# cvxgrp/qcqp

Measured on AMD Instinct MI355X. Metric: restarts x coord-sweeps / sec (improve COORD_DESCENT phase-2 sweeps, 2n^2 flops each; whole step timed), higher is better.
Workload: dtype f64

## Files before the change

### qcqp_amd/csrc/capi.hip

```cpp
#include <dlfcn.h>
#include <unistd.h>
#include <hip/hip_runtime.h>
#include <rccl/rccl.h>

#include <algorithm>
#include <cmath>
#include <cstdarg>
#include <cstdio>
#include <cstring>
#include <string>
#include <chrono>
#include <vector>

#include "../../include/qcqp_mi.h"
#include "kernels_impl.h"
#include "admm.h"
#include "admm_fused.h"
#include "cd_queue.h"
#include "cd_life.h"
#include "cd_small.h"
#include "admm_small.h"
#include "sdr_small.h"
#include "gemm_pk.h"
#include "cd_general.h"
// ... 112 lines not shown
    size_t h_pin_cap = 0;
    int64_t out_cap = 0;
    int eval_zs = 1;
    double *d_wS = nullptr, *d_wY = nullptr, *d_ww = nullptr, *d_wz = nullptr;
    int64_t wY_cap = 0;
    double *d_planes = nullptr;
    int64_t planes_cap = 0;
    double *d_gP = nullptr;
    const double *dn_Gpack = nullptr, *dn_q = nullptr, *dn_qT = nullptr, *dn_r = nullptr;
    const int *dn_relop = nullptr;
    double *dn_G = nullptr, *dn_Dg = nullptr, *dn_Ft = nullptr;
    int dense_chain_mode = 0;
    long long *dn_prof = nullptr;
    int64_t dn_G_cap = 0, dn_state_cap = 0;
    void *dn_state = nullptr;
    hipStream_t stream2 = nullptr;
    hipEvent_t dn_ev[3] = {nullptr, nullptr, nullptr};
    hipEvent_t dn_evn[2] = {nullptr, nullptr};
    int *dn_hn = nullptr;
    bool dn_force = false;
    double stream_limit = 16e9;
    double *dn_gp_pre = nullptr, *dn_tmp = nullptr;
    ncclComm_t comm = nullptr;
    int rank = 0, world = 1;
    double *d_comm = nullptr, *d_comm_big = nullptr;
    size_t comm_big_cap = 0;
    long long *d_prof = nullptr;
    int cd_stage = 0;
    int64_t Xi_cap = 0;
    bool sdr_factor_resident = false;
    double ad_Minv_rho = 0.0;
    bool ad_Minv_device = false;
    const char *last_cd2_kernel = "";
    bool profile = false;
    int dbg = 0;
    char *af_work = nullptr;
    size_t af_work_cap = 0;
    bool ad_fused = true;
    int ad_fused_nt = 512;
    const char *last_admm_kernel = "";
    int last_admm_C = 0;
    long long af_prof[16] = {0};
    int cd_queue = 2;
    int *d_qnext = nullptr;
    bool q_prepared = false;
    CdLife *d_life = nullptr;
    int Kreal = 0;
    double fbound = 0.0;
    double *l2_scratch = nullptr; size_t l2_scratch_cap = 0;
    double *l2_D = nullptr, *l2_S = nullptr;
    int *l2_abort = nullptr;
    int *l2_cuslot = nullptr;
    double *l2_preslack = nullptr; int64_t l2_preslack_cap = 0;
    double *lr_L = nullptr, *lr_G = nullptr, *lr_U = nullptr; int lr_RB = 0;
    int life_version = 0;
    long long *d_life_prof = nullptr;
    int64_t *d_bestK_idx = nullptr; double *d_bestK_key = nullptr, *d_bestK_x = nullptr; int64_t bestK_cap = 0;
    bool cd_ref_order = false;
    bool force_generic = false;
    std::vector<int> last_st1, last_st2;
    char *sb_work = nullptr;
    size_t sb_work_cap = 0;
    std::vector<double> unit_d;
    char *ss_work = nullptr;
    size_t ss_work_cap = 0;
};

namespace {

void admm_free(qcqpmi_ctx *c, bool keep_zsolver);

int fail(qcqpmi_ctx *c, int code, const char *fmt, ...) {
    char buf[1024];
    va_list ap;
    va_start(ap, fmt);
    vsnprintf(buf, sizeof(buf), fmt, ap);
    va_end(ap);
    if (c) c->err = buf; else g_create_error = buf;
    return code;
}

#define HIPCHK(c, expr)                                                                       \
    do {                                                                                      \
        hipError_t e_ = (expr);                                                               \
        if (e_ != hipSuccess)                                                                 \
            return fail(c, QCQPMI_EHIP, "%s failed: %s (%s:%d)", #expr, hipGetErrorString(e_), \
                        __FILE__, __LINE__);                                                  \
    } while (0)

template <typename T>
int dev_alloc(qcqpmi_ctx *c, T **p, size_t count, bool zero = true) {
    void *v = nullptr;
    HIPCHK(c, hipMalloc(&v, std::max<size_t>(count, 1) * sizeof(T)));
    if (zero) HIPCHK(c, hipMemsetAsync(v, 0, std::max<size_t>(count, 1) * sizeof(T), c->stream));
    *p = (T *)v;
    return 0;
}

template <typename T>
int prob_upload(qcqpmi_ctx *c, const T **dst, const std::vector<T> &src) {
    T *p = nullptr;
    int rc = dev_alloc(c, &p, src.size(), false);
    if (rc) return rc;
    c->prob_allocs.push_back(p);
    if (!src.empty())
        HIPCHK(c, hipMemcpyAsync(p, src.data(), src.size() * sizeof(T), hipMemcpyHostToDevice, c->stream));
// ... 425 lines not shown
}

#include "capi_small.inc"


extern "C" {

int qcqpmi_abi_version(void) { return QCQPMI_ABI_VERSION; }

int qcqpmi_device_count(void) {
    int n = 0;
    if (hipGetDeviceCount(&n) != hipSuccess) return 0;
    return n;
}

const char *qcqpmi_last_error(const qcqpmi_ctx *ctx) {
    return ctx ? ctx->err.c_str() : g_create_error.c_str();
}

int qcqpmi_ctx_create(qcqpmi_ctx **out, int64_t n, int64_t m, int device) {
    if (!out || n <= 0 || m < 0) return fail(nullptr, QCQPMI_EINVAL, "ctx_create: bad arguments");
    int ndev = qcqpmi_device_count();
    if (ndev <= 0)
        return fail(nullptr, QCQPMI_EHIP, "no HIP device visible: the qcqp_amd engine requires an MI355X (there is no CPU fallback)");
    if (device < 0 || device >= ndev) return fail(nullptr, QCQPMI_EINVAL, "device %d out of range (%d visible)", device, ndev);
    qcqpmi_ctx *c = new qcqpmi_ctx();
    c->device = device; c->n = n; c->m = m; c->n16 = (n + 15) / 16 * 16;
    c->quads.resize((size_t)m + 1);
    if (const char *sl = getenv("QCQPMI_STREAM_LIMIT")) { const double v = atof(sl); if (v > 0.0) c->stream_limit = v; }
    hipError_t e = hipSetDevice(device);
    if (e == hipSuccess) e = hipStreamCreateWithFlags(&c->stream, hipStreamNonBlocking);
    for (int i = 0; i < 5 && e == hipSuccess; i++) {
        e = hipEventCreate(&c->timers[i].beg);
        if (e == hipSuccess) e = hipEventCreate(&c->timers[i].end);
    }
    if (e != hipSuccess) {
        int rc = fail(nullptr, QCQPMI_EHIP, "ctx_create: %s", hipGetErrorString(e));
        delete c;
        return rc;
    }
    *out = c;
    return 0;
}

void qcqpmi_ctx_destroy(qcqpmi_ctx *c) {
    if (!c) return;
    (void)hipSetDevice(c->device);
    if (c->stream) (void)spin_sync(c->stream);
    if (c->comm && rccl() && rccl()->CommDestroy) rccl()->CommDestroy(c->comm);
    free_population(c);
    admm_free(c, false);
    for (void *p : c->prob_allocs) (void)hipFree(p);
    void *ptrs[] = {c->d_Fpack, c->d_Frow, c->d_mu, c->d_best_idx, c->d_best_key, c->d_comm, c->d_comm_big,
                    c->dn_G, c->dn_Dg, c->dn_Ft, c->dn_prof, c->dn_state, c->d_planes, c->d_out, c->d_wS, c->d_wY, c->d_ww, c->d_wz, c->af_work, c->d_qnext, c->d_life, c->d_life_prof, c->d_bestK_idx, c->d_bestK_key, c->d_bestK_x, c->l2_scratch, c->l2_D, c->l2_S, c->l2_abort, c->l2_cuslot, c->l2_preslack, c->lr_L, c->lr_G, c->lr_U, c->sb_work, c->ss_work};
    if (c->h_out) (void)hipHostFree(c->h_out);
    if (c->h_pin) (void)hipHostFree(c->h_pin);
    for (void *p : ptrs) if (p) (void)hipFree(p);
    for (auto &t : c->timers) { if (t.beg) (void)hipEventDestroy(t.beg); if (t.end) (void)hipEventDestroy(t.end); }
    for (auto &e : c->dn_ev) if (e) (void)hipEventDestroy(e);
    for (auto &e : c->dn_evn) if (e) (void)hipEventDestroy(e);
    if (c->dn_hn) (void)hipHostFree(c->dn_hn);
    if (c->stream2) (void)hipStreamDestroy(c->stream2);
    if (c->stream) (void)hipStreamDestroy(c->stream);
    delete c;
}

int qcqpmi_set_quad(qcqpmi_ctx *c, int64_t k, int format, const double *vals, const int64_t *idx,
                    const int64_t *ptr, int64_t nnz, const double *q, double r, int relop) {
    if (!c) return QCQPMI_EINVAL;
    if (c->finalized) return fail(c, QCQPMI_ESTATE, "set_quad after finalize");
    if (k < 0 || k > c->m || !q) return fail(c, QCQPMI_EINVAL, "set_quad: bad k or q");
    if ((k == 0) != (relop == 0) || relop < 0 || relop > 2)
        return fail(c, QCQPMI_EINVAL, "set_quad: relop %d invalid for function %lld", relop, (long long)k);
    HostQuad &h = c->quads[(size_t)k];
    h = HostQuad();
    const int64_t n = c->n;
    if (format == QCQPMI_FMT_DENSE) {
        if (!vals) return fail(c, QCQPMI_EINVAL, "set_quad: dense vals missing");
        for (int64_t i = 0; i < n; i++)
            for (int64_t j = 0; j < n; j++) {
                double v = vals[i * n + j];
                if (v != 0.0) { h.ci.push_back((int)i); h.cj.push_back((int)j); h.cv.push_back(v); }
            }
    } else if (format == QCQPMI_FMT_CSR) {
        if (!ptr || (nnz > 0 && (!idx || !vals))) return fail(c, QCQPMI_EINVAL, "set_quad: CSR arrays missing");
        for (int64_t i = 0; i < n; i++)
            for (int64_t e = ptr[i]; e < ptr[i + 1]; e++) {
                if (idx[e] < 0 || idx[e] >= n || e >= nnz) return fail(c, QCQPMI_EINVAL, "set_quad: CSR index out of range");
                if (vals[e] != 0.0) { h.ci.push_back((int)i); h.cj.push_back((int)idx[e]); h.cv.push_back(vals[e]); }
            }
    } else {
        return fail(c, QCQPMI_EINVAL, "set_quad: unknown format %d", format);
    }
    if (format == QCQPMI_FMT_DENSE) {
        for (int64_t i = 0; i < n; i++)
            for (int64_t j = i + 1; j < n; j++)
                if (vals[i * n + j] != vals[j * n + i])
                    return fail(c, QCQPMI_EINVAL, "set_quad: P of function %lld is not symmetric (entry %lld,%lld); pass (P + P^T)/2",
                                (long long)k, (long long)i, (long long)j);
    } else {
        std::vector<std::pair<int64_t, double>> ent(h.cv.size());
        for (size_t e = 0; e < h.cv.size(); e++) ent[e] = {(int64_t)h.ci[e] * n + h.cj[e], h.cv[e]};
        std::sort(ent.begin(), ent.end(), [](const std::pair<int64_t, double> &a, const std::pair<int64_t, double> &b) { return a.first < b.first; });
        size_t w = 0;
        for (size_t e = 0; e < ent.size(); e++) {
            if (w > 0 && ent[w - 1].first == ent[e].first) ent[w - 1].second += ent[e].second;
            else ent[w++] = ent[e];
// ... 653 lines not shown
            a.prof = c->d_prof;
        }
        bool used_rs = false;
        a.f0out = c->d_f0; a.mvout = c->d_mv;
        rc = (c->maxc <= 1) ? launch_cd<1>(c, a, false, used_lds, &used_rs) : launch_cd<4>(c, a, false, used_lds, &used_rs);
        if (rc) return rc;
        if (!used_rs && (rc = launch_eval(c, false))) return rc;
        if (stage == 2) { c->cd_stage = 2; return 0; }
    }
    c->cd_stage = 0;
    std::vector<int> st, st1;
    if ((rc = fetch_cd_outputs(c, sweeps1, sweeps2, visits2, accepted2, ran_phase2, f0, maxviol, st, st1))) return rc;
    if ((rc = cd_apply_status(c, st, st1, f0, maxviol, 0))) return rc;
    return 0;
}

int qcqpmi_cd_run(qcqpmi_ctx *c, int phase1, int64_t num_iters, double viol_tol, double tol,
                  uint64_t seed, uint64_t first_index, int64_t *sweeps1, int64_t *sweeps2,
                  int64_t *visits2, int64_t *accepted2, uint8_t *ran_phase2, double *f0,
                  double *maxviol) {
    return qcqpmi_cd_run_stage(c, 0, phase1, num_iters, viol_tol, tol, seed, first_index, sweeps1, sweeps2, visits2, accepted2,
                               ran_phase2, f0, maxviol);
}

int qcqpmi_cd_dense_block_step(qcqpmi_ctx *c, int phase, int64_t sweep, int64_t block, int coord_lo, int coord_hi, double viol_tol,
                               double tol, uint64_t seed, uint64_t first_index, const double *slack) {
    int rc = check_ready(c, true);
    if (rc) return rc;
    if (!dense_on(c)) return fail(c, QCQPMI_EUNSUPPORTED, "cd_dense_block_step: the problem does not take the dense-constraint path");
    c->last_cd2_kernel = dense_chain_name(c);
    return cd_dense_block_step(c, phase, sweep, block, coord_lo, coord_hi, viol_tol, tol, seed, first_index, slack);
}

static int cd_life2_reserve(qcqpmi_ctx *c, int nmw, int cus) {
    int rc;
    const size_t need = (size_t)cd_life2_max_wgs(nmw, cus, 1) * (size_t)c->n16 * 16;
    if (need > c->l2_scratch_cap) {
        if (c->l2_scratch) { HIPCHK(c, spin_sync(c->stream)); (void)hipFree(c->l2_scratch); c->l2_scratch = nullptr; c->l2_scratch_cap = 0; }
        if ((rc = dev_alloc(c, &c->l2_scratch, need))) return rc;
        c->l2_scratch_cap = need;
    }
    if (!c->l2_abort && (rc = dev_alloc(c, &c->l2_abort, 4))) return rc;
    if (!c->l2_cuslot && (rc = dev_alloc(c, &c->l2_cuslot, 4096))) return rc;
    if (!c->l2_D) {
        const size_t NB = (size_t)(c->n16 / 16);
        if ((rc = dev_alloc(c, &c->l2_D, NB * 256))) return rc;
        if ((rc = dev_alloc(c, &c->l2_S, NB * 48))) return rc;
        hipError_t e = (hipError_t)cd_life2_pack(c->dp, c->l2_D, c->l2_S, c->stream);
        if (e != hipSuccess) return fail(c, QCQPMI_EHIP, "cd_life2_pack: %s", hipGetErrorString(e));
    }
    return 0;
}

int qcqpmi_cd_stream_run(qcqpmi_ctx *c, int64_t K, int64_t R, int generate, int phase1, int64_t num_iters, double viol_tol, double tol,
                         uint64_t seed, uint64_t seed_stride, uint64_t first_index, uint64_t first_stride, double select_tol,
                         int64_t *sweeps1, int64_t *sweeps2, int64_t *visits2, int64_t *accepted2, uint8_t *ran_phase2, double *f0,
                         double *maxviol, int64_t *best_index, double *best_f0, double *best_maxviol, double *best_x) {
    int rc = check_ready(c, generate ? false : true);
    if (rc) return rc;
    if (K < 1 || R < 1 || num_iters < 0 || !(tol > 0.0) || K * R >= (1LL << 30)) return fail(c, QCQPMI_EINVAL, "cd_stream_run: bad K / R / num_iters / tol");
    if (!generate && c->R != K * R) return fail(c, QCQPMI_EINVAL, "cd_stream_run: the resident population has %lld points, K R = %lld", (long long)c->R, (long long)(K * R));
    HIPCHK(c, hipSetDevice(c->device));
    const bool stt = getenv("QCQPMI_STREAM_TIMING") != nullptr;
    double stm[6] = {0, 0, 0, 0, 0, 0};
    auto stnow = []() { return std::chrono::duration<double, std::milli>(std::chrono::steady_clock::now().time_since_epoch()).count(); };
    stm[0] = stnow();
    int nmw = 0, cs2 = 0, kind = 0;
    const int factor_rb = (c->lr_RB > 0 && c->life_version != 3 && cd_life2_factor_ok(c->dp, 16 * (int64_t)c->lr_RB)) ? c->lr_RB : 0;
    bool use2 = c->life_version != 1 && !c->force_generic && !(c->dbg & 64) && c->sep &&
                cd_life2_config(c->dp, c->Kreal, c->objclass, c->symcls, factor_rb, &nmw, &cs2, &kind);
    int cs = 0;
    const int queue_switch = c->cd_queue;
    c->cd_queue = 2;
    const bool eligible = cd_queue_eligible(c, false) && (int)(c->n16 / 16) - 4 <= RQ_NSIMD * RQ_MAXU && c->n16 >= 48;
    c->cd_queue = queue_switch;
    const bool lr = use2 && factor_rb > 0 && nmw == 3 && (kind == L2_KIND_BAND || kind == L2_KIND_GEN);
    if (lr) cs2 = 0;
    if (!use2) {
        if (!eligible || c->life_version != 1)
            return fail(c, QCQPMI_EUNSUPPORTED, "cd_stream_run: the lifecycle kernel needs separable constraints -- at most four classes of coordinates, at most two constraints "
                        "per coordinate --, a diagonal of P0 that is positive everywhere or zero everywhere (a diagonal of mixed sign: ONE class with one constraint "
                        "per coordinate only; with several classes or two constraints per coordinate it runs the serial path), and 33 <= n <= 2304: use qcqpmi_cd_run "
                        "per population");
        const int NBq = (int)(c->n16 / 16);
        cs = (c->dbg & 128) ? ((c->dbg >> 8) & 7) : 4;
        cs = cs > RQ_CSMAX ? RQ_CSMAX : cs;
        if (cs >= NBq) cs = 0;
        cs &= ~1;
        if (NBq - cs > RQ_NSIMD * RQ_MAXU || NBq < 3) return fail(c, QCQPMI_EUNSUPPORTED, "cd_stream_run: n = %lld outside the range of cd_phase2_qs_kernel (n <= 1024, at least 3 blocks of 16)", (long long)c->n);
    }
    if (generate && (rc = pop_reserve(c, K * R))) return rc;
    if (!c->d_qnext && (rc = dev_alloc(c, &c->d_qnext, 16))) return rc;
    if (!c->d_life) HIPCHK(c, hipMalloc((void **)&c->d_life, sizeof(CdLife)));
    HIPCHK(c, hipMemsetAsync(c->d_qnext, 0, 16 * sizeof(int), c->stream));
    CdLife L;
    L.on = 1; L.generate = generate ? 1 : 0; L.phase1 = phase1 ? 1 : 0; L.Rtotal = K * R; L.Rpop = R;
    L.seed = seed; L.seed_stride = seed_stride; L.first_index = first_index; L.first_stride = first_stride; L.viol_tol = viol_tol;
    L.sweeps1 = c->d_sweeps1; L.status1 = c->d_status1; L.ran2 = c->d_flag;
    L.prof = nullptr;
    const char *pre_ev = getenv("QCQPMI_L2_PREBUILT");
    const bool pre = lr && !(pre_ev && atoi(pre_ev) == 0);
    L.prebuilt = pre ? 1 : 0; L.preslack = nullptr;
    if (pre) {
        if (K * R > c->l2_preslack_cap) {
            if (c->l2_preslack) { HIPCHK(c, spin_sync(c->stream)); (void)hipFree(c->l2_preslack); c->l2_preslack = nullptr; c->l2_preslack_cap = 0; }
            if ((rc = dev_alloc(c, &c->l2_preslack, (size_t)(K * R)))) return rc;
            c->l2_preslack_cap = K * R;
        }
        L.preslack = c->l2_preslack;
    }
    if (c->profile) {
        if (!c->d_life_prof) HIPCHK(c, hipMalloc((void **)&c->d_life_prof, 24 * sizeof(long long)));
        HIPCHK(c, hipMemsetAsync(c->d_life_prof, 0, 24 * sizeof(long long), c->stream));
        L.prof = c->d_life_prof;
    }
    HIPCHK(c, hipMemcpyAsync(c->d_life, &L, sizeof(L), hipMemcpyHostToDevice, c->stream));
    HIPCHK(c, spin_sync(c->stream));
    int cus = 0;
    HIPCHK(c, hipDeviceGetAttribute(&cus, hipDeviceAttributeMultiprocessorCount, c->device));
    stm[1] = stnow();
    if (use2) {
        if ((rc = cd_life2_reserve(c, nmw, cus))) return rc;
        if (!lr && (c->dbg & 128)) { const int k2 = (c->dbg >> 8) & 7; if (nmw == 3 && (k2 == 0 || k2 == 2 || k2 == 4) && k2 < (int)(c->n16 / 16)) cs2 = k2; }
        const int tiles = cd_life2_tiles(c->dp, nmw, cs2, K * R, cus, 0, lr ? 1 : 0);
        int64_t wgs = (K * R + 16 * tiles - 1) / (16 * tiles);
        const int maxw = cd_life2_max_wgs(nmw, cus, tiles);
        if (wgs > maxw) wgs = maxw;
        if (c->dbg & 1024) { const int lim = (c->dbg >> 12) & 1023; if (lim > 0 && wgs > lim) wgs = lim; }
        CdLife2Args qa;
        qa.P = c->dp; qa.num_iters = num_iters; qa.tol = tol; qa.life = c->d_life;
        cd_queue_fill_batch(c, qa.b, seed, first_index);
        qa.b.R = K * R;
        qa.scratch = c->l2_scratch; qa.Dpack = c->l2_D; qa.Spack = c->l2_S; qa.abort = c->l2_abort; qa.fbound = c->fbound;
        { const char *ev = getenv("QCQPMI_L2_ROT"); const int rot = ev ? atoi(ev) : (lr ? 2 : 0); qa.cuslot = rot ? c->l2_cuslot : nullptr; qa.rotmode = rot; }
        if (qa.cuslot) HIPCHK(c, hipMemsetAsync(c->l2_cuslot, 0, 4096 * sizeof(int), c->stream));
        qa.dbg = (c->dbg & 2048) ? 1 : 0;
        qa.Gpack = lr ? c->lr_G : nullptr; qa.Upack = lr ? c->lr_U : nullptr; qa.RB = lr ? c->lr_RB : 0;
        qa.nclass = c->Kreal;
        const double l0 = stnow();
        (void)hipEventRecord(c->timers[2].beg, c->stream);
        const double l1 = stnow();
        hipError_t qe = pre ? (hipError_t)cd_life2_prep_launch(c->dp, c->d_life, c->X, K * R, num_iters, tol, c->stream) : hipSuccess;
        if (qe == hipSuccess) qe = (hipError_t)cd_life2_launch(qa, nmw, cs2, kind, tiles, (int)wgs, c->stream);
        const double l2 = stnow();
        (void)hipEventRecord(c->timers[2].end, c->stream);
        c->timers[2].valid = true;
        if (qe != hipSuccess) return fail(c, QCQPMI_EHIP, "cd_stream_run: %s", hipGetErrorString(qe));
        c->last_cd2_kernel = cd_life2_name(nmw, kind, tiles, lr ? 1 : 0);
        int ab = 0;
        HIPCHK(c, spin_sync(c->stream));
        const double l3 = stnow();
        HIPCHK(c, hipMemcpyAsync(&ab, c->l2_abort, sizeof(int), hipMemcpyDeviceToHost, c->stream));
        const double l4 = stnow();
        HIPCHK(c, spin_sync(c->stream));
        if (stt) fprintf(stderr, "cd_stream_run launch (ms): reserve %.3f, event %.3f, launch call %.3f, event + spin wait %.3f, copy call %.3f, sync %.3f\n", l0 - stm[1], l1 - l0, l2 - l1, l3 - l2, l4 - l3, stnow() - l4);
        if (ab) {
            HIPCHK(c, hipMemsetAsync(c->l2_abort, 0, sizeof(int), c->stream));
            c->R = 0;
            return fail(c, QCQPMI_EHIP, "cd_stream_run: a wait inside cd_life_kernel ran into its watchdog (internal error; no results)");
        }
    } else {
        CdQueueArgs qa;
        qa.P = c->dp; qa.num_iters = num_iters; qa.tol = tol;
        qa.life = c->d_life; qa.life_on = 1;
        cd_queue_fill_batch(c, qa.b, seed, first_index);
        qa.b.R = K * R;
        (void)hipEventRecord(c->timers[2].beg, c->stream);
        hipError_t qe = (hipError_t)cd_queue_launch(qa, cs, cus, c->stream);
        (void)hipEventRecord(c->timers[2].end, c->stream);
        c->timers[2].valid = true;
        if (qe != hipSuccess) return fail(c, QCQPMI_EHIP, "cd_stream_run: %s", hipGetErrorString(qe));
        HIPCHK(c, spin_sync(c->stream));
        c->last_cd2_kernel = "cd_phase2_qs_kernel<lifecycle>";
    }
    c->cd_stage = 0;
    c->evaluated = true;
    if (stt) { (void)spin_sync(c->stream); stm[2] = stnow(); }
    std::vector<int> st, st1;
    if ((rc = fetch_cd_outputs(c, sweeps1, sweeps2, visits2, accepted2, ran_phase2, f0, maxviol, st, st1))) return rc;
    stm[3] = stnow();
    if ((rc = cd_apply_status(c, st, st1, f0, maxviol, 0))) return rc;
    stm[4] = stnow();
    if (best_index || best_f0 || best_maxviol || best_x) {
        if ((rc = cd_bestK_reserve(c, K))) return rc;
        hipLaunchKernelGGL(select_best_kernel, dim3((unsigned)K), dim3(1024), 0, c->stream, (const double *)c->d_f0, (const double *)c->d_mv,
                           R, select_tol, c->d_bestK_idx, c->d_bestK_key);
        if (best_x) {
            HIPCHK(c, hipMemsetAsync(c->d_bestK_x, 0, (size_t)K * c->n * sizeof(double), c->stream));
            hipLaunchKernelGGL(gather_best_x_kernel, dim3((unsigned)K), dim3(256), 0, c->stream, (const double *)c->X, c->n, c->n16, R,
                               (const int64_t *)c->d_bestK_idx, c->d_bestK_x);
        }
        HIPCHK(c, hipGetLastError());
        std::vector<int64_t> idx((size_t)K * 2);
        std::vector<double> key((size_t)K * 2);
        HIPCHK(c, hipMemcpyAsync(idx.data(), c->d_bestK_idx, idx.size() * sizeof(int64_t), hipMemcpyDeviceToHost, c->stream));
        HIPCHK(c, hipMemcpyAsync(key.data(), c->d_bestK_key, key.size() * sizeof(double), hipMemcpyDeviceToHost, c->stream));
        if (best_x) HIPCHK(c, hipMemcpyAsync(best_x, c->d_bestK_x, (size_t)K * c->n * sizeof(double), hipMemcpyDeviceToHost, c->stream));
        HIPCHK(c, spin_sync(c->stream));
        for (int64_t p = 0; p < K; p++) {
            if (best_index) best_index[p] = idx[(size_t)2 * p];
            if (best_f0) best_f0[p] = key[(size_t)2 * p];
            if (best_maxviol) best_maxviol[p] = key[(size_t)2 * p + 1];
        }
    }
    if (stt) {
        stm[5] = stnow();
        fprintf(stderr, "cd_stream_run timing (ms): set-up %.3f, launch + kernel %.3f, fetch %.3f, status %.3f, best %.3f\n", stm[1] - stm[0], stm[2] - stm[1],
                stm[3] - stm[2], stm[4] - stm[3], stm[5] - stm[4]);
    }
    return 0;
}

int qcqpmi_cd_stream_reserve(qcqpmi_ctx *c, int64_t K, int64_t R) {
    int rc = check_ready(c, false);
    if (rc) return rc;
    if (K < 1 || R < 1 || K * R >= (1LL << 30)) return fail(c, QCQPMI_EINVAL, "cd_stream_reserve: bad K / R");
    HIPCHK(c, hipSetDevice(c->device));
    if (K * R > c->Rcap) { if ((rc = pop_reserve(c, K * R))) return rc; }
    if ((rc = cd_outputs_reserve(c, K * R))) return rc;
    if ((rc = cd_bestK_reserve(c, K))) return rc;
    if (!c->d_qnext && (rc = dev_alloc(c, &c->d_qnext, 16))) return rc;
    if (!c->d_life) HIPCHK(c, hipMalloc((void **)&c->d_life, sizeof(CdLife)));
    {
        int nmw = 0, cs2 = 0, kind = 0, cus = 0;
        HIPCHK(c, hipDeviceGetAttribute(&cus, hipDeviceAttributeMultiprocessorCount, c->device));
        if (c->life_version != 1 && c->sep && cd_life2_config(c->dp, c->Kreal, c->objclass, c->symcls, c->lr_RB, &nmw, &cs2, &kind) && (rc = cd_life2_reserve(c, nmw, cus))) return rc;
    }
    return 0;
}

int qcqpmi_debug_life_profile(qcqpmi_ctx *c, int64_t *out16) {
    if (!c || !out16) return QCQPMI_EINVAL;
    for (int k = 0; k < 24; k++) out16[k] = 0;
    if (!c->d_life_prof) return 0;
    HIPCHK(c, hipSetDevice(c->device));
    HIPCHK(c, spin_sync(c->stream));
    HIPCHK(c, hipMemcpy(out16, c->d_life_prof, 24 * sizeof(long long), hipMemcpyDeviceToHost));
    return 0;
}

int qcqpmi_cd_status(qcqpmi_ctx *c, int *status1, int *status2) {
    if (!c) return QCQPMI_EINVAL;
    if ((int64_t)c->last_st1.size() != c->R || (int64_t)c->last_st2.size() != c->R)
        return fail(c, QCQPMI_ESTATE, "cd_status: no coordinate-descent run on the resident population");
    if (status1) memcpy(status1, c->last_st1.data(), (size_t)c->R * sizeof(int));
    if (status2) memcpy(status2, c->last_st2.data(), (size_t)c->R * sizeof(int));
    return 0;
}


int qcqpmi_select_best(qcqpmi_ctx *c, double tol, int64_t *best_index, double *best_f0,
                       double *best_maxviol, double *best_x) {
    int rc = check_ready(c, true);
    if (rc) return rc;
    HIPCHK(c, hipSetDevice(c->device));
    if (!c->evaluated && (rc = launch_eval(c, false))) return rc;
    hipLaunchKernelGGL(select_best_kernel, dim3(1), dim3(1024), 0, c->stream, c->d_f0, c->d_mv, c->R, tol,
                       c->d_best_idx, c->d_best_key);
    HIPCHK(c, hipGetLastError());
    int64_t idx[2];
    double key[2];
    HIPCHK(c, hipMemcpyAsync(idx, c->d_best_idx, sizeof(idx), hipMemcpyDeviceToHost, c->stream));
    HIPCHK(c, hipMemcpyAsync(key, c->d_best_key, sizeof(key), hipMemcpyDeviceToHost, c->stream));
    HIPCHK(c, spin_sync(c->stream));
    if (best_index) *best_index = idx[0];
    if (best_f0) *best_f0 = key[0];
    if (best_maxviol) *best_maxviol = key[1];
    if (best_x && idx[0] >= 0) {
        int64_t r = idx[0];
        const double *src = c->X + (r >> 4) * c->n16 * 16 + (r & 15);
        HIPCHK(c, hipMemcpy2DAsync(best_x, sizeof(double), src, 16 * sizeof(double), sizeof(double), (size_t)c->n,
                                   hipMemcpyDeviceToHost, c->stream));
        HIPCHK(c, spin_sync(c->stream));
    }
    return 0;
}

const char *qcqpmi_last_cd_kernel(qcqpmi_ctx *c) { return c ? c->last_cd2_kernel : ""; }

// ... 204 lines not shown
```

### qcqp_amd/csrc/cd_life.h

```cpp
#pragma once
#include <hip/hip_runtime.h>
#include <stdint.h>
#include "kernels.h"
#include "cd_queue.h"

namespace qcqpmi {

enum { L2_KIND_BAND = 0, L2_KIND_GEN = 1, L2_KIND_LIN = 2, L2_KIND_GENK = 3, L2_KIND_LINK = 4, L2_KIND_SGN = 5 };

struct CdLife2Args {
    DevProblem P;
    CdBatch b;
    int64_t num_iters;
    double tol;
    const CdLife *life;
    double *scratch;
    const double *Dpack;
    const double *Spack;
    int *abort;
    int *cuslot;
    double fbound;
    const double *Gpack, *Upack;
    int RB;
    int rotmode;
    int nclass;
    int dbg;
};

bool cd_life2_config(const DevProblem &P, int Kreal, int objclass, bool symcls, int factor_rb, int *nmw, int *cs, int *kind);
size_t cd_life2_lds_bytes(int nmw, int cs, int tiles, int lr, int kind);
bool cd_life2_factor_ok(const DevProblem &P, int64_t r);
int cd_life2_pack_factor(const double *Lrow, double *Gpack, double *Upack, int NB, int RB, hipStream_t st);
int cd_life2_max_wgs(int nmw, int cus, int tiles);
int cd_life2_tiles(const DevProblem &P, int nmw, int cs, int64_t restarts, int cus, int requested, int lr);
int cd_life2_pack(const DevProblem &P, double *Dpack, double *Spack, hipStream_t st);
int cd_life2_prep_launch(const DevProblem &P, const CdLife *life, double *X, int64_t Rtotal, int64_t num_iters, double tol, hipStream_t st);
int cd_life2_launch(const CdLife2Args &a, int nmw, int cs, int kind, int tiles, int wgs, hipStream_t st);
const char *cd_life2_name(int nmw, int kind, int tiles, int lr);

}
```

### qcqp_amd/csrc/cd_life.hip

```cpp
#include "cd_life.h"

#include <cstdio>
#include <cstdlib>

#include "onevar.h"
#include "cd_phase1_sep.h"
#include "cd_chain.h"
#include "cd_roles.h"

namespace qcqpmi {
namespace {

constexpr int L2_WD = 1 << 21;
enum { L2_ABORT = 3 };

__device__ __attribute__((always_inline)) inline RqOwn l2_own(int NB, int CS, int m, int NMW) {
    RqOwn o;
    const int rest = NB - CS;
    o.NB = NB;
    if (m < 0) { o.first = rest; o.stride = 1; o.nu = CS; }
    else { o.first = m; o.stride = NMW; o.nu = m < rest ? (rest - m + NMW - 1) / NMW : 0; }
    return o;
}

// ... 1099 lines not shown
                double v = -QM_INF;
                for (int64_t i = tid; i < P.n; i += NT) {
                    const double x = Xg[i * 16 + cc];
                    if (MULTI) {
                        for (int e = P.cptr[i]; e < P.cptr[i + 1]; e++) {
                            const double f = (P.cp[e] * x + P.cq[e]) * x + P.cr[e];
                            const double w = viol_of(f, P.crel[e]);
                            v = w > v ? w : v;
                        }
                    } else {
                        const double f = (cp * x + cq) * x + cr;
                        const double w = (rel == RELOP_EQ) ? fabs(f) : (f > 0.0 ? f : 0.0);
                        v = w > v ? w : v;
                    }
                }
                v = wave_max(v);
                if (lane == 0) atomicMax(&l2_tl(p1key, ct, TD)[cc], ordered_key(v));
            }
            __syncthreads();
            if (tid < NS && l2_tl(snew, tid >> 4, TD)[tid & 15]) {
                const int st = tid >> 4, sc = tid & 15;
                double mvx;
                if (lf_pre) {
                    const int id = l2_tl(sid, st, TD)[sc];
                    mvx = glb(lf->preslack)[id];
                    l2_tl(p1sw, st, TD)[sc] = (int)glb(lf->sweeps1)[id];
                    l2_tl(p1st, st, TD)[sc] = glb(lf->status1)[id];
                    l2_tl(gatep, st, TD)[sc] = glb(lf->ran2)[id];
                } else {
                    mvx = ordered_unkey(l2_tl(p1key, st, TD)[sc]);
                    l2_tl(gatep, st, TD)[sc] = (mvx < lf_viol_tol && l2_tl(p1st, st, TD)[sc] == 0) ? 1 : 0;
                }
                l2_tl(slk, st, TD)[sc] = mvx;
                L2_STORE_SETS(st, sc, mvx)
            }
            __syncthreads();
            if (nlast < 16) {
                for (int w = tid; w < NS * (16 - nlast); w += NT) {
                    const int c = w % NS, ct = c >> 4, cc = c & 15, row = w / NS;
                    if (l2_tl(snew, ct, TD)[cc] || l2_tl(sid, ct, TD)[cc] < 0) {
                        const int nn = l2_tl(TC.n, ct, TD)[cc];
                        double xp = 0.0;
                        if (BK == L2_KIND_BAND) xp = nn >= 2 ? l2_tl(TC.lo, ct, TD)[16 * KCLV + cc] : 0.0;
                        else if (BK == L2_KIND_GEN) xp = nn >= 1 ? l2_tl(TC.hi, ct, TD)[cc] : 0.0;
                        else xp = nn >= 2 ? l2_tl(TC.hi, ct, TD)[16 * KCLV + cc] : l2_tl(TC.hi, ct, TD)[cc];
                        if (!(xp == xp) || __builtin_isinf(xp)) xp = 0.0;
                        (Xg0 + (int64_t)ct * n16 * 16)[(P.n + row) * 16 + cc] = xp;
                    }
                }
                __syncthreads();
            }
            if (LR) {
                const int r16 = 16 * a0.RB;
                for (int w = tid; w < NS * (32 + r16); w += NT) {
                    const int c = w % NS, ct = c >> 4, cc = c & 15, rowz = w / NS;
                    if (l2_tl(snew, ct, TD)[cc] || l2_tl(sid, ct, TD)[cc] < 0) {
                        if (rowz < 32) l2_tl(pend, ct, TD)[rowz * 16 + cc] = 0.0;
                        else l2_tl(ytile, ct, TD)[(rowz - 32) * 16 + cc] = 0.0;
                    }
                }
                __syncthreads();
            }
            if (lf->prof && tid == 0) {
                int nn = 0;
                for (int k = 0; k < NS; k++) nn += l2_tl(snew, k >> 4, TD)[k & 15] ? 1 : 0;
                atomicAdd((unsigned long long *)lf->prof + 0, (unsigned long long)((long long)__builtin_amdgcn_s_memtime() - pt0));
                atomicAdd((unsigned long long *)lf->prof + 2, 1ull);
                atomicAdd((unsigned long long *)lf->prof + 3, (unsigned long long)nn);
            }
            __builtin_amdgcn_s_setprio(0);
        }
        if (role == 0) {
            long long *cs_ = l2_tl(cst, rtile, TD);
            if (l2_tl(snew, rtile, TD)[r]) {
#pragma unroll
                for (int f = 0; f < 6; f++) cs_[f * 64 + lane] = 0;
                const int pass = l2_tl(gatep, rtile, TD)[r];
                cs_[6 * 64 + lane] = 0;
                cs_[4 * 64 + lane] = (pass && !PRE && !LR) ? 0 : 1;
                cs_[7 * 64 + lane] = (pass ? (PRE ? 4 : 0) : 1) | (LR ? 8 : 0);
                cs_[8 * 64 + lane] = 0;
            } else if (l2_tl(sid, rtile, TD)[r] < 0) {
                cs_[4 * 64 + lane] = 1; cs_[6 * 64 + lane] = 0;
                cs_[7 * 64 + lane] = 2; cs_[8 * 64 + lane] = 0;
            }
        }
        __syncthreads();
        if (tid == 0 && glb(lifep)->prof) *(long long *)(ctl + 6) = (long long)__builtin_amdgcn_s_memtime();

        if (role > 0) {
            if (LR) l2_mfma_lr_role<NMW>(role - 1, rtile);
            else l2_mfma_role<NMW, CS>(role - 1, rtile);
        } else l2_chain_role<NMW, CS, KIND, TILES, LR>(rtile);

        __syncthreads();
        if (sy[L2_ABORT] || (TILES > 1 && l2_tl((int *)sy, 1, TD)[L2_ABORT])) {
            if (tid == 0) __hip_atomic_store(glb(a0.abort), 1, __ATOMIC_RELAXED, __HIP_MEMORY_SCOPE_AGENT);
            break;
        }
        if (tid == 0 && glb(lifep)->prof)
        {
            const long long now_ = (long long)__builtin_amdgcn_s_memtime();
            atomicAdd((unsigned long long *)glb(lifep)->prof + 5, (unsigned long long)(now_ - *(long long *)(ctl + 6)));
            atomicAdd((unsigned long long *)glb(lifep)->prof + 20, (unsigned long long)(now_ - *(long long *)(ctl + 8)));
        }
        {
            const int e0 = P.cptr[P.krep[0]];
            const double cp = P.cp[e0], cq = P.cq[e0], cr = P.cr[e0];
            const int rel = P.crel[e0];
            if (tid == 0) { int cnt = 0; for (int k = 0; k < NS; k++) if (l2_tl(sfin, k >> 4, TD)[k & 15]) p1cols[cnt++] = k; ctl[4] = cnt; }
            if (tid < NS) l2_tl(p1key, tid >> 4, TD)[tid & 15] = ordered_key(-QM_INF);
            __syncthreads();
            const int nfin = ctl[4];
            const int64_t items = (int64_t)nfin * n16;
            for (int64_t w0 = tid; w0 < items; w0 += (int64_t)NT * 8) {
                double xv8[8];
#pragma unroll
                for (int u = 0; u < 8; u++) {
                    const int64_t w = w0 + (int64_t)NT * u;
                    const int col = p1cols[w < items ? w / n16 : 0];
                    const int64_t i = w % n16;
                    xv8[u] = (w < items && i < P.n) ? (Xg0 + (int64_t)(col >> 4) * n16 * 16)[i * 16 + (col & 15)] : 0.0;
                }
#pragma unroll
                for (int u = 0; u < 8; u++) {
                    const int64_t w = w0 + (int64_t)NT * u;
                    if (w < items) {
                        const int col = p1cols[w / n16], id = l2_tl(sid, col >> 4, TD)[col & 15];
                        const int64_t i = w % n16;
                        glb(a0.b.X)[((int64_t)(id >> 4) * n16 + i) * 16 + (id & 15)] = xv8[u];
                        if (i < P.n) {
                            if (MULTI) {
                                double vv = -QM_INF;
// ... 93 lines not shown
                            }
                    } else {
                        for (int64_t i = j; i < j + 2 && i < n; i++) {
                            int fl = 0;
                            double v = 0.0;
                            const double xi = p1_class_visit(cp, cq, cr, rel, i, Xt[16 * i], tol, viol_tol, sd, gidx, t, &fl, &v);
                            if (fl & 1) { Xt[16 * i] = xi; moved = 1; }
                            if (fl >> 8) stv = -(fl >> 8);
                            va = v > va ? v : va;
                        }
                    }
                }
            }
#pragma unroll
            for (int o = 16; o <= 32; o <<= 1) {
                const double w = __shfl_xor(va, o, 64);
                va = w > va ? w : va;
                moved |= __shfl_xor(moved, o, 64);
            }
            if ((tid & 63) < 16 && !fin[s]) { atomicMax(&key[s], ordered_key(va)); if (moved) upd[s] = 1; }
            if (stv) st1[s] = stv;
            __syncthreads();
            if (tid < 16 && !fin[tid]) {
                sw[tid]++;
                if (ordered_unkey(key[tid]) < viol_tol || !upd[tid]) fin[tid] = 1;
            }
        }
    }
    __syncthreads();
    if (tid < 16) key[tid] = ordered_key(-QM_INF);
    __syncthreads();
    double v = -QM_INF;
    if (valid)
        for (int64_t j = 2 * g; j < n; j += 32)
            for (int64_t i = j; i < j + 2 && i < n; i++) {
                const double x = Xt[16 * i];
                const double f = (cp * x + cq) * x + cr;
                const double w = (rel == RELOP_EQ) ? fabs(f) : (f > 0.0 ? f : 0.0);
                v = w > v ? w : v;
            }
#pragma unroll
    for (int o = 16; o <= 32; o <<= 1) { const double w = __shfl_xor(v, o, 64); v = w > v ? w : v; }
    if ((tid & 63) < 16 && valid) atomicMax(&key[s], ordered_key(v));
    __syncthreads();
    if (tid < 16 && valid) {
        const double mvx = ordered_unkey(key[tid]);
        glb(const_cast<double *>(lf->preslack))[id] = mvx;
        glb(lf->sweeps1)[id] = sw[tid];
        glb(lf->status1)[id] = st1[tid];
        glb(lf->ran2)[id] = (mvx < viol_tol && st1[tid] == 0) ? 1 : 0;
    }
}

__global__ void l2_pack_kernel(DevProblem P, double *Dpack, double *Spack) {
    const int b = blockIdx.x, t = threadIdx.x;
    const int64_t n16 = P.n16;
    const int rr = t >> 4, cc = t & 15;
    Dpack[(int64_t)b * 256 + t] = (cc > rr) ? P.P0[(16 * (int64_t)b + rr) * n16 + 16 * b + cc] : 0.0;
    if (t < 16) {
        const int64_t i = 16 * (int64_t)b + t;
        const double d = P.P0[i * n16 + i], rc = P.rcp2d[i];
        Spack[(int64_t)b * 48 + t] = 0.5 * P.q0[i];
        Spack[(int64_t)b * 48 + 16 + t] = rc + rc;
        Spack[(int64_t)b * 48 + 32 + t] = d;
    }
}

__global__ void l2_pack_factor_kernel(const double *__restrict__ L, double *__restrict__ Gpack, double *__restrict__ Upack, int NB, int RB) {
    const int64_t idx = (int64_t)blockIdx.x * blockDim.x + threadIdx.x;
    if (idx >= (int64_t)NB * RB * 256) return;
    const int e = (int)(idx & 1), lane = (int)((idx >> 1) & 63), vp = (int)((idx >> 7) & 1);
    const int64_t rest = idx >> 8;
    const int beta = (int)(rest % RB), b = (int)(rest / RB), v = 2 * vp + e;
    const int64_t r16 = 16 * (int64_t)RB;
    Gpack[idx] = L[(16 * (int64_t)b + (lane & 15)) * r16 + 16 * beta + 4 * v + (lane >> 4)];
    Upack[idx] = L[(16 * (int64_t)b + 4 * v + (lane >> 4)) * r16 + 16 * beta + (lane & 15)];
}

template <int NMW, int CS, int TILES, int LR>
int l2_launch_kind(const CdLife2Args &a, int kind, int wgs, size_t lds, hipStream_t st) {
    constexpr bool MK = TILES == 1 && !LR;
    if (!MK && (kind == L2_KIND_GENK || kind == L2_KIND_LINK)) return (int)hipErrorInvalidValue;
    if (LR && kind == L2_KIND_SGN) return (int)hipErrorInvalidValue;
    auto k = kind == L2_KIND_SGN ? cd_life_kernel<NMW, CS, LR ? L2_KIND_GEN : L2_KIND_SGN, TILES, LR> : kind == L2_KIND_BAND ? cd_life_kernel<NMW, CS, L2_KIND_BAND, TILES, LR> : (kind == L2_KIND_GEN || LR) ? cd_life_kernel<NMW, CS, L2_KIND_GEN, TILES, LR>
             : kind == L2_KIND_GENK ? cd_life_kernel<NMW, CS, MK ? L2_KIND_GENK : L2_KIND_GEN, TILES, LR>
             : kind == L2_KIND_LINK ? cd_life_kernel<NMW, CS, MK ? L2_KIND_LINK : L2_KIND_GEN, TILES, LR>
                                    : cd_life_kernel<NMW, CS, LR ? L2_KIND_GEN : L2_KIND_LIN, TILES, LR>;
    hipError_t e = hipFuncSetAttribute((const void *)k, hipFuncAttributeMaxDynamicSharedMemorySize, (int)lds);
    if (e != hipSuccess) return (int)e;
    hipLaunchKernelGGL(k, dim3((unsigned)wgs), dim3((NMW == 3 && TILES == 1) ? 256 : 512), lds, st, a);
    return (int)hipGetLastError();
}

}

size_t cd_life2_lds_bytes(int nmw, int cs, int tiles, int lr, int kind) {
    const bool multi = kind == L2_KIND_GENK || kind == L2_KIND_LINK;
    return ((size_t)L2_SHARED_DOUBLES + (size_t)tiles * (size_t)l2_tile_doubles(nmw, cs > 0 ? cs : 1, lr, multi ? L2_KCL : 1, multi ? 2 : 1)) * sizeof(double) + 256;
}

bool cd_life2_factor_ok(const DevProblem &P, int64_t r) {
    const int64_t r16 = (r + 15) / 16 * 16;
    if (r < 1 || r16 > 16 * L2_YBMAX || P.NB < 8) return false;
    return true;
}

int cd_life2_pack_factor(const double *Lrow, double *Gpack, double *Upack, int NB, int RB, hipStream_t st) {
    const int64_t tot = (int64_t)NB * RB * 256;
    hipLaunchKernelGGL(l2_pack_factor_kernel, dim3((unsigned)((tot + 255) / 256)), dim3(256), 0, st, Lrow, Gpack, Upack, NB, RB);
    return (int)hipGetLastError();
}

int cd_life2_prep_launch(const DevProblem &P, const CdLife *life, double *X, int64_t Rtotal, int64_t num_iters, double tol, hipStream_t st) {
    hipLaunchKernelGGL(cd_life_prep_kernel, dim3((unsigned)((Rtotal + 15) / 16)), dim3(L2P_NT), 0, st, P, life, X, num_iters, tol);
    return (int)hipGetLastError();
}

int cd_life2_max_wgs(int nmw, int cus, int tiles) { return (nmw == 3 && tiles == 1) ? 2 * cus : cus; }

bool cd_life2_config(const DevProblem &P, int Kreal, int objclass, bool symcls, int factor_rb, int *nmw, int *cs, int *kind) {
    if (!P.sep || P.maxc < 1 || P.maxc > 2 || Kreal < 1 || Kreal > L2_KCL) return false;
    const bool multi = P.maxc > 1 || Kreal > 1;
    if (objclass != 0 && objclass != 1 && objclass != 2) return false;
    if (objclass == 0 && multi) return false;
    const int NB = (int)P.NB;
    if (NB < 3) return false;
    int w, c;
    if (NB <= 4) { w = 3; c = 0; }
    else if (NB - 4 <= 3 * RQ_MAXU) { w = 3; c = (NB < 8) ? 2 : 4; }
    else if (factor_rb > 0 && !multi && objclass == 1 && NB <= 256) { w = 3; c = 0; }
    else if (NB - 4 <= 7 * RQ_MAXU) { w = 7; c = 4; }
    else return false;
    *nmw = w; *cs = c;
    *kind = objclass == 0 ? L2_KIND_SGN : multi ? (objclass == 2 ? L2_KIND_LINK : L2_KIND_GENK) : objclass == 2 ? L2_KIND_LIN : (symcls ? L2_KIND_BAND : L2_KIND_GEN);
    return true;
}

int cd_life2_tiles(const DevProblem &P, int nmw, int cs, int64_t restarts, int cus, int requested, int lr) {
    (void)P; (void)restarts; (void)cus;
    if (!lr || nmw != 3 || cs != 0) return 1;
    int t = requested;
    if (const char *ev = getenv("QCQPMI_L2_TILES")) t = atoi(ev);
    return t == 2 ? 2 : 1;
}

int cd_life2_pack(const DevProblem &P, double *Dpack, double *Spack, hipStream_t st) {
    hipLaunchKernelGGL(l2_pack_kernel, dim3((unsigned)P.NB), dim3(256), 0, st, P, Dpack, Spack);
    return (int)hipGetLastError();
}

int cd_life2_launch(const CdLife2Args &a, int nmw, int cs, int kind, int tiles, int wgs, hipStream_t st) {
    const int lr = a.RB > 0 ? 1 : 0;
    if (const char *ev = getenv("QCQPMI_L2_CS")) {
        const int k2 = atoi(ev);
        if (!lr && nmw == 3 && tiles == 1 && (k2 == 0 || k2 == 2 || k2 == 4) && k2 + 3 <= (int)a.P.NB && (int)a.P.NB - k2 <= 3 * RQ_MAXU) cs = k2;
    }
    const size_t lds = cd_life2_lds_bytes(nmw, cs, tiles, lr, kind);
    if (getenv("QCQPMI_L2_DEBUG")) {
        int occ = -1;
        hipError_t e = lr ? (tiles == 2 ? hipOccupancyMaxActiveBlocksPerMultiprocessor(&occ, cd_life_kernel<3, 0, L2_KIND_BAND, 2, 1>, 512, lds)
                                        : hipOccupancyMaxActiveBlocksPerMultiprocessor(&occ, cd_life_kernel<3, 0, L2_KIND_BAND, 1, 1>, 256, lds))
                     : nmw == 3 ? hipOccupancyMaxActiveBlocksPerMultiprocessor(&occ, cd_life_kernel<3, 4, L2_KIND_BAND, 1, 0>, 256, lds)
                                : hipOccupancyMaxActiveBlocksPerMultiprocessor(&occ, cd_life_kernel<7, 4, L2_KIND_BAND, 1, 0>, 512, lds);
        fprintf(stderr, "cd_life2_launch: nmw %d cs %d kind %d tiles %d lr %d wgs %d lds %zu: occupancy %d workgroups per CU (%s)\n", nmw, cs, kind, tiles, lr, wgs, lds, occ, hipGetErrorString(e));
    }
    if (wgs < 1) wgs = 1;
    if (lr) {
// ... 27 lines not shown
```

### qcqp_amd/csrc/cd_queue.h

```cpp
#pragma once
#include <hip/hip_runtime.h>
#include <stdint.h>
#include "kernels.h"

namespace qcqpmi {

struct CdBatch {
    double *X;
    const double *f0cur;
    const double *slack;
    const uint8_t *flag;
    int64_t *visits, *accepted, *sweeps;
    int *status;
    double *f0out, *mvout;
    int64_t R;
    uint64_t seed, first_index;
    int *next;
};

struct CdLife {
    int on;
    int generate;
    int phase1;
    int64_t Rtotal, Rpop;
    uint64_t seed, seed_stride, first_index, first_stride;
    double viol_tol;
    int64_t *sweeps1;
    int *status1;
    uint8_t *ran2;
    long long *prof;
    int prebuilt;
    const double *preslack;
};

struct CdQueueArgs {
    DevProblem P;
    CdBatch b;
    int64_t num_iters;
    double tol;
    const CdLife *life;
    int life_on;
};

size_t cd_queue_lds_bytes(const DevProblem &P);
int cd_queue_launch(const CdQueueArgs &a, int cs, int max_wgs, hipStream_t st);

}
```

Before: 28.21 million.

## Precompute low-rank factor projections Y0 with a batched MFMA kernel before CD

Adds a separate kernel that computes the initial low-rank projection Y0 = U^T x for all restarts up front, using f64 MFMA over tiles of restarts and factor blocks. The persistent CD kernel then seeds its pend/ytile state from the precomputed Y0 and pending X rows instead of zeroing them and rebuilding them in-kernel with the load path. This replaces per-restart serial initialization inside the lifecycle kernel with a dense batched GEMM-like pass. In exchange it needs up to a 2 GiB buffer, an extra launch and an extra global-memory round trip.

New measurement: 28.74 million, median of 6. +1.9%, better.

```diff
diff --git a/qcqp_amd/csrc/capi.hip b/qcqp_amd/csrc/capi.hip
--- a/qcqp_amd/csrc/capi.hip
+++ b/qcqp_amd/csrc/capi.hip
@@ -188,6 +188,7 @@
     int *l2_abort = nullptr;
     int *l2_cuslot = nullptr;
     double *l2_preslack = nullptr; int64_t l2_preslack_cap = 0;
+    double *l2_y0 = nullptr; size_t l2_y0_cap = 0;
     double *lr_L = nullptr, *lr_G = nullptr, *lr_U = nullptr; int lr_RB = 0;
     int life_version = 0;
     long long *d_life_prof = nullptr;
@@ -719,7 +720,7 @@
     admm_free(c, false);
     for (void *p : c->prob_allocs) (void)hipFree(p);
     void *ptrs[] = {c->d_Fpack, c->d_Frow, c->d_mu, c->d_best_idx, c->d_best_key, c->d_comm, c->d_comm_big,
-                    c->dn_G, c->dn_Dg, c->dn_Ft, c->dn_prof, c->dn_state, c->d_planes, c->d_out, c->d_wS, c->d_wY, c->d_ww, c->d_wz, c->af_work, c->d_qnext, c->d_life, c->d_life_prof, c->d_bestK_idx, c->d_bestK_key, c->d_bestK_x, c->l2_scratch, c->l2_D, c->l2_S, c->l2_abort, c->l2_cuslot, c->l2_preslack, c->lr_L, c->lr_G, c->lr_U, c->sb_work, c->ss_work};
+                    c->dn_G, c->dn_Dg, c->dn_Ft, c->dn_prof, c->dn_state, c->d_planes, c->d_out, c->d_wS, c->d_wY, c->d_ww, c->d_wz, c->af_work, c->d_qnext, c->d_life, c->d_life_prof, c->d_bestK_idx, c->d_bestK_key, c->d_bestK_x, c->l2_scratch, c->l2_D, c->l2_S, c->l2_abort, c->l2_cuslot, c->l2_preslack, c->l2_y0, c->lr_L, c->lr_G, c->lr_U, c->sb_work, c->ss_work};
     if (c->h_out) (void)hipHostFree(c->h_out);
     if (c->h_pin) (void)hipHostFree(c->h_pin);
     for (void *p : ptrs) if (p) (void)hipFree(p);
@@ -1479,6 +1480,30 @@
     return 0;
 }
 
+constexpr int64_t L2_Y0_BUDGET = (int64_t)2 << 30;
+static int64_t cd_life2_y0_count(int64_t KR, int RB) {
+    int64_t cnt = KR;
+    if (const char *ev = getenv("QCQPMI_L2_Y0_MAX")) { const long long m = atoll(ev); cnt = m < 0 ? 0 : (m < cnt ? m : cnt); }
+    const int64_t fit = L2_Y0_BUDGET / ((int64_t)RB * 16 * 16 * (int64_t)sizeof(double)) * 16;
+    return cnt < fit ? cnt : fit;
+}
+
+static int cd_life2_pre_reserve(qcqpmi_ctx *c, int64_t KR, int RB) {
+    int rc;
+    if (KR > c->l2_preslack_cap) {
+        if (c->l2_preslack) { HIPCHK(c, spin_sync(c->stream)); (void)hipFree(c->l2_preslack); c->l2_preslack = nullptr; c->l2_preslack_cap = 0; }
+        if ((rc = dev_alloc(c, &c->l2_preslack, (size_t)KR))) return rc;
+        c->l2_preslack_cap = KR;
+    }
+    const size_t need = (size_t)((cd_life2_y0_count(KR, RB) + 15) / 16) * (size_t)RB * 256;
+    if (need > c->l2_y0_cap) {
+        if (c->l2_y0) { HIPCHK(c, spin_sync(c->stream)); (void)hipFree(c->l2_y0); c->l2_y0 = nullptr; c->l2_y0_cap = 0; }
+        if ((rc = dev_alloc(c, &c->l2_y0, need, false))) return rc;
+        c->l2_y0_cap = need;
+    }
+    return 0;
+}
+
 int qcqpmi_cd_stream_run(qcqpmi_ctx *c, int64_t K, int64_t R, int generate, int phase1, int64_t num_iters, double viol_tol, double tol,
                          uint64_t seed, uint64_t seed_stride, uint64_t first_index, uint64_t first_stride, double select_tol,
                          int64_t *sweeps1, int64_t *sweeps2, int64_t *visits2, int64_t *accepted2, uint8_t *ran_phase2, double *f0,
@@ -1528,14 +1553,14 @@
     const char *pre_ev = getenv("QCQPMI_L2_PREBUILT");
     const bool pre = lr && !(pre_ev && atoi(pre_ev) == 0);
     L.prebuilt = pre ? 1 : 0; L.preslack = nullptr;
+    L.y0_count = 0; L.y0 = nullptr;
     if (pre) {
-        if (K * R > c->l2_preslack_cap) {
-            if (c->l2_preslack) { HIPCHK(c, spin_sync(c->stream)); (void)hipFree(c->l2_preslack); c->l2_preslack = nullptr; c->l2_preslack_cap = 0; }
-            if ((rc = dev_alloc(c, &c->l2_preslack, (size_t)(K * R)))) return rc;
-            c->l2_preslack_cap = K * R;
-        }
+        if ((rc = cd_life2_pre_reserve(c, K * R, factor_rb))) return rc;
         L.preslack = c->l2_preslack;
-    }
+        L.y0_count = cd_life2_y0_count(K * R, factor_rb);
+        L.y0 = c->l2_y0;
+    }
+    const int64_t y0_count = L.y0_count;
     if (c->profile) {
         if (!c->d_life_prof) HIPCHK(c, hipMalloc((void **)&c->d_life_prof, 24 * sizeof(long long)));
         HIPCHK(c, hipMemsetAsync(c->d_life_prof, 0, 24 * sizeof(long long), c->stream));
@@ -1568,6 +1593,8 @@
         (void)hipEventRecord(c->timers[2].beg, c->stream);
         const double l1 = stnow();
         hipError_t qe = pre ? (hipError_t)cd_life2_prep_launch(c->dp, c->d_life, c->X, K * R, num_iters, tol, c->stream) : hipSuccess;
+        if (qe == hipSuccess && y0_count > 0)
+            qe = (hipError_t)cd_life2_y0_launch(c->X, c->lr_U, c->l2_y0, (int)(c->n16 / 16), factor_rb, c->n16, y0_count, c->stream);
         if (qe == hipSuccess) qe = (hipError_t)cd_life2_launch(qa, nmw, cs2, kind, tiles, (int)wgs, c->stream);
         const double l2 = stnow();
         (void)hipEventRecord(c->timers[2].end, c->stream);
@@ -1652,6 +1679,11 @@
         int nmw = 0, cs2 = 0, kind = 0, cus = 0;
         HIPCHK(c, hipDeviceGetAttribute(&cus, hipDeviceAttributeMultiprocessorCount, c->device));
         if (c->life_version != 1 && c->sep && cd_life2_config(c->dp, c->Kreal, c->objclass, c->symcls, c->lr_RB, &nmw, &cs2, &kind) && (rc = cd_life2_reserve(c, nmw, cus))) return rc;
+        const int factor_rb = (c->lr_RB > 0 && c->life_version != 3 && cd_life2_factor_ok(c->dp, 16 * (int64_t)c->lr_RB)) ? c->lr_RB : 0;
+        const bool lr = factor_rb > 0 && c->life_version != 1 && !c->force_generic && !(c->dbg & 64) && c->sep &&
+                        cd_life2_config(c->dp, c->Kreal, c->objclass, c->symcls, factor_rb, &nmw, &cs2, &kind) && nmw == 3 && (kind == L2_KIND_BAND || kind == L2_KIND_GEN);
+        const char *pre_ev = getenv("QCQPMI_L2_PREBUILT");
+        if (lr && !(pre_ev && atoi(pre_ev) == 0) && (rc = cd_life2_pre_reserve(c, K * R, factor_rb))) return rc;
     }
     return 0;
 }
diff --git a/qcqp_amd/csrc/cd_life.h b/qcqp_amd/csrc/cd_life.h
--- a/qcqp_amd/csrc/cd_life.h
+++ b/qcqp_amd/csrc/cd_life.h
@@ -35,6 +35,7 @@
 int cd_life2_tiles(const DevProblem &P, int nmw, int cs, int64_t restarts, int cus, int requested, int lr);
 int cd_life2_pack(const DevProblem &P, double *Dpack, double *Spack, hipStream_t st);
 int cd_life2_prep_launch(const DevProblem &P, const CdLife *life, double *X, int64_t Rtotal, int64_t num_iters, double tol, hipStream_t st);
+int cd_life2_y0_launch(const double *X, const double *Upack, double *Y0, int NB, int RB, int64_t n16, int64_t count, hipStream_t st);
 int cd_life2_launch(const CdLife2Args &a, int nmw, int cs, int kind, int tiles, int wgs, hipStream_t st);
 const char *cd_life2_name(int nmw, int kind, int tiles, int lr);
 
diff --git a/qcqp_amd/csrc/cd_life.hip b/qcqp_amd/csrc/cd_life.hip
--- a/qcqp_amd/csrc/cd_life.hip
+++ b/qcqp_amd/csrc/cd_life.hip
@@ -1175,11 +1175,18 @@
             }
             if (LR) {
                 const int r16 = 16 * a0.RB;
+                const int y0n = lf_pre ? (int)lf->y0_count : 0;
+                GLB const double *y0g = glb(lf->y0);
                 for (int w = tid; w < NS * (32 + r16); w += NT) {
                     const int c = w % NS, ct = c >> 4, cc = c & 15, rowz = w / NS;
-                    if (l2_tl(snew, ct, TD)[cc] || l2_tl(sid, ct, TD)[cc] < 0) {
-                        if (rowz < 32) l2_tl(pend, ct, TD)[rowz * 16 + cc] = 0.0;
-                        else l2_tl(ytile, ct, TD)[(rowz - 32) * 16 + cc] = 0.0;
+                    const int id = l2_tl(sid, ct, TD)[cc];
+                    if (l2_tl(snew, ct, TD)[cc] || id < 0) {
+                        double v = 0.0;
+                        if (id >= 0 && id < y0n)
+                            v = rowz < 32 ? (Xg0 + (int64_t)ct * n16 * 16)[(16 * (int64_t)(NB - 2) + rowz) * 16 + cc]
+                                          : y0g[((int64_t)(id >> 4) * r16 + (rowz - 32)) * 16 + (id & 15)];
+                        if (rowz < 32) l2_tl(pend, ct, TD)[rowz * 16 + cc] = v;
+                        else l2_tl(ytile, ct, TD)[(rowz - 32) * 16 + cc] = v;
                     }
                 }
                 __syncthreads();
@@ -1199,9 +1206,14 @@
 #pragma unroll
                 for (int f = 0; f < 6; f++) cs_[f * 64 + lane] = 0;
                 const int pass = l2_tl(gatep, rtile, TD)[r];
+                bool load = LR != 0;
+                if (LR) {
+                    GLB const CdLife *lf = glb(lifep);
+                    if (lf->prebuilt && l2_tl(sid, rtile, TD)[r] < (int)lf->y0_count) load = false;
+                }
                 cs_[6 * 64 + lane] = 0;
-                cs_[4 * 64 + lane] = (pass && !PRE && !LR) ? 0 : 1;
-                cs_[7 * 64 + lane] = (pass ? (PRE ? 4 : 0) : 1) | (LR ? 8 : 0);
+                cs_[4 * 64 + lane] = (pass && !PRE && !load) ? 0 : 1;
+                cs_[7 * 64 + lane] = (pass ? (PRE ? 4 : 0) : 1) | (load ? 8 : 0);
                 cs_[8 * 64 + lane] = 0;
             } else if (l2_tl(sid, rtile, TD)[r] < 0) {
                 cs_[4 * 64 + lane] = 1; cs_[6 * 64 + lane] = 0;
@@ -1401,6 +1413,71 @@
     }
 }
 
+constexpr int L2Y_NT = 256, L2Y_BW = 4, L2Y_TW = 4;
+__global__ __launch_bounds__(L2Y_NT, 2) void cd_life_y0_kernel(const double *__restrict__ X, const double *__restrict__ Upack, double *__restrict__ Y0,
+                                                               int NB, int RB, int ntiles, int64_t n16) {
+    const int lane = threadIdx.x & 63;
+    const int wave = __builtin_amdgcn_readfirstlane((int)(threadIdx.x >> 6));
+    const int nbg = (RB + L2Y_BW - 1) / L2Y_BW;
+    const int64_t gw = (int64_t)blockIdx.x * (L2Y_NT / 64) + wave;
+    const int beta0 = (int)(gw % nbg) * L2Y_BW;
+    const int64_t t0 = gw / nbg * L2Y_TW;
+    if (t0 >= ntiles) return;
+    GLB const v2d_ *ua[L2Y_BW];
+    GLB const double *xt[L2Y_TW];
+#pragma unroll
+    for (int u = 0; u < L2Y_BW; u++) ua[u] = (GLB const v2d_ *)glb(Upack) + (int64_t)(beta0 + u < RB ? beta0 + u : RB - 1) * 128 + lane;
+#pragma unroll
+    for (int k = 0; k < L2Y_TW; k++) xt[k] = glb(X) + (t0 + k < ntiles ? t0 + k : (int64_t)ntiles - 1) * n16 * 16 + lane;
+    v4d_ y[L2Y_BW][L2Y_TW];
+#pragma unroll
+    for (int u = 0; u < L2Y_BW; u++)
+#pragma unroll
+        for (int k = 0; k < L2Y_TW; k++) y[u][k] = v4d_{0.0, 0.0, 0.0, 0.0};
+    const int nblk = NB - 2;
+    v2d_ a[L2Y_BW][2];
+    double x[L2Y_TW][4];
+#pragma unroll
+    for (int u = 0; u < L2Y_BW; u++) { a[u][0] = ua[u][0]; a[u][1] = ua[u][64]; }
+#pragma unroll
+    for (int k = 0; k < L2Y_TW; k++)
+#pragma unroll
+        for (int v = 0; v < 4; v++) x[k][v] = xt[k][v * 64];
+    for (int b = 0; b < nblk; b++) {
+        const int bn = b + 1 < nblk ? b + 1 : b;
+        v2d_ an[L2Y_BW][2];
+        double xn[L2Y_TW][4];
+#pragma unroll
+        for (int u = 0; u < L2Y_BW; u++) { an[u][0] = ua[u][(int64_t)bn * RB * 128]; an[u][1] = ua[u][(int64_t)bn * RB * 128 + 64]; }
+#pragma unroll
+        for (int k = 0; k < L2Y_TW; k++)
+#pragma unroll
+            for (int v = 0; v < 4; v++) xn[k][v] = xt[k][(int64_t)bn * 256 + v * 64];
+#pragma unroll
+        for (int v = 0; v < 4; v++)
+#pragma unroll
+            for (int u = 0; u < L2Y_BW; u++)
+#pragma unroll
+                for (int k = 0; k < L2Y_TW; k++) y[u][k] = __builtin_amdgcn_mfma_f64_16x16x4f64(a[u][v >> 1][v & 1], x[k][v], y[u][k], 0, 0, 0);
+#pragma unroll
+        for (int u = 0; u < L2Y_BW; u++) { a[u][0] = an[u][0]; a[u][1] = an[u][1]; }
+#pragma unroll
+        for (int k = 0; k < L2Y_TW; k++)
+#pragma unroll
+            for (int v = 0; v < 4; v++) x[k][v] = xn[k][v];
+    }
+    const int64_t r16 = 16 * (int64_t)RB;
+#pragma unroll
+    for (int u = 0; u < L2Y_BW; u++)
+#pragma unroll
+        for (int k = 0; k < L2Y_TW; k++)
+            if (beta0 + u < RB && t0 + k < ntiles) {
+                GLB double *dst = glb(Y0) + ((t0 + k) * r16 + 16 * (beta0 + u)) * 16 + lane;
+#pragma unroll
+                for (int v = 0; v < 4; v++) dst[v * 64] = y[u][k][v];
+            }
+}
+
 __global__ void l2_pack_kernel(DevProblem P, double *Dpack, double *Spack) {
     const int b = blockIdx.x, t = threadIdx.x;
     const int64_t n16 = P.n16;
@@ -1462,6 +1539,15 @@
 
 int cd_life2_prep_launch(const DevProblem &P, const CdLife *life, double *X, int64_t Rtotal, int64_t num_iters, double tol, hipStream_t st) {
     hipLaunchKernelGGL(cd_life_prep_kernel, dim3((unsigned)((Rtotal + 15) / 16)), dim3(L2P_NT), 0, st, P, life, X, num_iters, tol);
+    return (int)hipGetLastError();
+}
+
+int cd_life2_y0_launch(const double *X, const double *Upack, double *Y0, int NB, int RB, int64_t n16, int64_t count, hipStream_t st) {
+    if (count < 1) return (int)hipSuccess;
+    if (NB < 3 || RB < 1) return (int)hipErrorInvalidValue;
+    const int64_t ntiles = (count + 15) / 16;
+    const int64_t waves = (ntiles + L2Y_TW - 1) / L2Y_TW * ((RB + L2Y_BW - 1) / L2Y_BW);
+    hipLaunchKernelGGL(cd_life_y0_kernel, dim3((unsigned)((waves + L2Y_NT / 64 - 1) / (L2Y_NT / 64))), dim3(L2Y_NT), 0, st, X, Upack, Y0, NB, RB, (int)ntiles, n16);
     return (int)hipGetLastError();
 }
 
diff --git a/qcqp_amd/csrc/cd_queue.h b/qcqp_amd/csrc/cd_queue.h
--- a/qcqp_amd/csrc/cd_queue.h
+++ b/qcqp_amd/csrc/cd_queue.h
@@ -31,6 +31,8 @@
     long long *prof;
     int prebuilt;
     const double *preslack;
+    int64_t y0_count;
+    const double *y0;
 };
 
 struct CdQueueArgs {
```
